# IamJerryXu/Multimodal-Diagnosis-HAM-Spine

Hardware: AMD Instinct MI355X
Metric: training images/sec, ResNet50+BERT-base 224px bs32 (higher is better)
Workload: dtype bf16; 1 GPU; C2: ResNet50 + BERT-base(L=128) + cross-attention FusionModule + MLP head, 224x224, batch 32 per GPU, CE(label_smoothing=0.02), fused AdamW, train-mode BatchNorm and dropout; per_gpu_batch=32, global_batch=32, seq_len=128, params=134897991, parallelism=dp1

## Files before the change

### multimodal-diagnosis-ham-spine_amd/hamspine/csrc/blocks.hip

```cpp
#include <algorithm>
#include <mutex>
#include <unordered_map>
#include <vector>
#include <stdlib.h>
#include "hs_common.h"
#include "pw_stream.h"

namespace hs {

__global__ __launch_bounds__(256) void gather3_kernel(const float* __restrict__ a, const float* __restrict__ b,
                                                      const float* __restrict__ c, float* __restrict__ dst, int n) {
    const int i = blockIdx.x * 256 + threadIdx.x;
    if (i >= 3 * n) return;
    const int w = i / n, k = i - w * n;
    dst[i] = w == 0 ? a[k] : (w == 1 ? b[k] : c[k]);
}

int gemm_impl(const hs_gemm_params* p, hipStream_t stream);
int gemm_stat_rows(const hs_gemm_params* p);
int gemm_bn_finish_rows(const hs_gemm_params* p);
int gemm_tile_rows(const hs_gemm_params* p);
int gemm_bnb_finish_rows(const hs_gemm_params* p);
void gemm_group_set_immediate_hook(int (*fn)(void*), void* ctx);
struct GemmGroup;
GemmGroup* gemm_group_open(hipStream_t s, long long slot);
int gemm_group_add(GemmGroup* g, const hs_gemm_params* p, hipStream_t s, const int* k_cols = nullptr);
bool gemm_group_takes_k_cols();
int gemm_group_flush(GemmGroup* g, hipStream_t s);
bool fused_attention_enabled();
int attention_bwd_fused(const hs_attn_desc& d, const void* q, const void* k, const void* v, const void* dO, void* dq, void* dk,
                        void* dv, const void* P, int ldP, void* scratch, long long scratch_bytes, const void* O, hipStream_t s,
                        const int* cu);
int attention_fwd_fused(const hs_attn_desc& d, const void* q, const void* k, const void* v, void* o, void* P, void* Pd, int ldP,
                        hipStream_t s, const int* cu);
int ln_fwd(int dtype, const void* x, const float* gamma, const float* beta, void* y, float* mean, float* rstd, long long M, int H,
           float eps, hipStream_t s, const int* nrows);
int ln_bwd(int dtype, const void* dy, const void* x, const float* gamma, const float* mean, const float* rstd, void* dx, float* dgamma,
           float* dbeta, float* ws, long long ws_bytes, long long M, int H, hipStream_t s, const int* inv);
int ln_bwd_pre(int dtype, const void* dy, const void* x, const float* gamma, const float* mean, const float* rstd, void* dx,
               float* dgamma, float* dbeta, void* dx_dropped, float* dbias, float p, unsigned long long seed, float* ws,
               long long ws_bytes, long long M, int H, hipStream_t s, const int* inv);
// ... 167 lines not shown
        } else {
            ++m;
        }
    }
    return HS_OK;
}
static int milestones_flush(Run& r) {
    if (r.plan) return HS_OK;
    for (int m = 0; m < g_ms.n; ++m) HS_CHECK_HIP(hipEventRecord(g_ms.ev[m], r.s));
    g_ms.n = 0;
    return HS_OK;
}

static hs_gemm_params gemm_defaults(int dt) {
    hs_gemm_params p;
    memset(&p, 0, sizeof(p));
    p.dtype = dt;
    p.out_dtype = dt;
    p.alpha = 1.f;
    p.batch = 1;
    p.batch_inner = 1;
    return p;
}
static int gemm_splitk(Run& r, hs_gemm_params& p, bool may_defer = false) {
    const int split = hs_gemm_suggest_split(p.M, p.N, p.K, p.dtype);
    const long long mk = r.ws.mark();
    p.split_k = split;
    if (split > 1) p.splitk_ws = (float*)r.ws.alloc(hs_gemm_splitk_ws_bytes(&p));
    const bool defer = may_defer && r.defer_wgrad && p.dtype == HS_BF16;
    if (!r.plan) {
        if (r.ws.overflow) {
            set_error("gemm_splitk: workspace too small");
            return HS_ERR_ARG;
        }
        if (may_defer && (knock() & 1)) {
        } else if (defer) HS_PROPAGATE(gemm_group_add(p.b_kind == HS_B_CONV ? r.grp_conv : r.grp_pw, &p, r.s));
        else HS_PROPAGATE(gemm_impl(&p, r.s));
    }
    if (defer) return HS_OK;
    if (r.plan ? !overlap_enabled() : !r.side) r.ws.release(mk);
    return HS_OK;
}

struct AttnLayout {
    int ldP;
    void *P, *Pd;
    float* S;
    void* dS;
};
static AttnLayout attn_layout(const hs_attn_desc& d, Run& r, bool backward) {
    AttnLayout l;
    const long long BH = (long long)d.B * d.H;
    l.ldP = (int)align_up(d.Lk, 8);
    l.P = r.saved.alloc(BH * d.Lq * l.ldP * esize(d.dtype));
    l.Pd = d.dropout_p > 0.f ? r.saved.alloc(BH * d.Lq * l.ldP * esize(d.dtype)) : l.P;
    l.S = (float*)r.ws.alloc(BH * d.Lq * d.Lk * 4);
    l.dS = backward ? r.ws.alloc(BH * d.Lq * l.ldP * esize(d.dtype)) : nullptr;
    return l;
}
static int attn_check(const hs_attn_desc& d) {
// ... 366 lines not shown
}

struct ConvShape {
    int N, H, W, Cin, Cout, R, stride, pad, P, Q;
};
static ConvShape conv_shape(int N, int H, int W, const hs_conv_bn& c) {
    ConvShape s;
    s.N = N; s.H = H; s.W = W; s.Cin = c.Cin; s.Cout = c.Cout; s.R = c.R; s.stride = c.stride; s.pad = c.pad;
    s.P = (H + 2 * c.pad - c.R) / c.stride + 1;
    s.Q = (W + 2 * c.pad - c.R) / c.stride + 1;
    return s;
}
static hs_conv_geom geom_of(const ConvShape& s) {
    hs_conv_geom g;
    memset(&g, 0, sizeof(g));
    g.N = s.N; g.H = s.H; g.W = s.W; g.C = s.Cin; g.P = s.P; g.Q = s.Q; g.K = s.Cout; g.R = s.R; g.S = s.R;
    g.stride = s.stride; g.pad = s.pad;
    g.row_pitch = s.W * s.Cin;
    g.img_pitch = s.H * g.row_pitch;
    g.qstep = s.stride * s.Cin;
    return g;
}
static bool is_pointwise(const ConvShape& s) { return s.R == 1 && s.stride == 1 && s.pad == 0; }
static bool fused_ln_bwd_enabled() {
    static int v = -1;
    if (v < 0) {
        const char* e = getenv("HAMSPINE_FUSED_LN_BWD");
        v = (e && e[0] == '0') ? 0 : 1;
    }
    return v == 1;
}
static bool grouped_wgrad_enabled() {
    static int v = -1;
    if (v < 0) {
        const char* e = getenv("HAMSPINE_GROUPED_WGRAD");
        v = (e && e[0] == '0') ? 0 : 1;
    }
    return v == 1;
}
static bool bn_mask_from_x_enabled() {
    static int v = -1;
    if (v < 0) {
        const char* e = getenv("HAMSPINE_BN_MASK_FROM_X");
        v = (e && e[0] == '1') ? 1 : 0;
    }
    return v == 1;
// ... 87 lines not shown
struct BnSums {
    const void* c;
    const float *scale, *shift, *mean, *invstd;
    float* partials;
    long long partials_cap;
    int* rows;
    const void* y = nullptr;
    const hs_bn_bwd_params* finish = nullptr;
    int* done = nullptr;
};
static bool bnb_finish_enabled() {
    static const bool on = [] { const char* e = getenv("HAMSPINE_BNB_FINISH"); return e && e[0] == '1'; }();
    return on;
}
static bool fused_bn_bwd_enabled() {
    static int v = -1;
    if (v < 0) {
        const char* e = getenv("HAMSPINE_FUSED_BN_BWD");
        v = (e && e[0] == '0') ? 0 : 1;
    }
    return v == 1;
}
static int conv_dgrad_run(Run& r, const ConvShape& s, const void* dy, const void* w_c, void* dx, const void* residual,
                          const BnSums* bnb = nullptr) {
    hs_gemm_params p = gemm_defaults(r.dt);
    p.M = (int)((long long)s.N * s.H * s.W); p.N = s.Cin; p.K = s.R * s.R * s.Cout;
    p.A = dy; p.B = w_c;
    p.a_elems = (long long)s.N * s.P * s.Q * s.Cout;
    p.b_elems = (long long)s.Cout * s.R * s.R * s.Cin;
    p.D = dx; p.ldd = s.Cin;
    p.residual = residual; p.ldr = s.Cin;
    if (is_pointwise(s)) {
        p.a_kind = HS_A_KC; p.lda = s.Cout;
        p.b_kind = HS_B_RC; p.ldb = s.Cin;
    } else {
        p.a_kind = HS_A_DGRAD; p.b_kind = HS_B_WDGRAD; p.g = geom_of(s);
    }
    if (bnb && bnb->rows) *bnb->rows = 0;
    if (!r.plan && (knock() & 512)) return HS_OK;
    if (bnb && (!residual || bnb->y) && r.dt == HS_BF16 && s.stride == 1 && s.Cin % 8 == 0 && fused_bn_bwd_enabled() && !(knock() & 16)) {
        p.split_k = hs_gemm_suggest_split(p.M, p.N, p.K, p.dtype);
        hs_gemm_params probe = p;
        probe.bnb_x = bnb->c; probe.bnb_scale = bnb->scale; probe.bnb_shift = bnb->shift; probe.bnb_mean = bnb->mean;
        probe.bnb_invstd = bnb->invstd; probe.bnb_partials = bnb->partials; probe.bnb_y = bnb->y;
        const int rows = r.plan ? 0 : gemm_tile_rows(&probe);
        if (bnb->done) *bnb->done = 0;
        if (rows > 0 && ((long long)rows * s.Cin * 2 + 4ll * s.Cin) * 4 <= bnb->partials_cap) {
            p = probe;
            *bnb->rows = rows;
            const int frows = (bnb->finish && bnb->done && bnb_finish_enabled()) ? gemm_bnb_finish_rows(&probe) : 0;
            if (frows > 0 && ((long long)frows * s.Cin * 2 + 4ll * s.Cin) * 4 <= bnb->partials_cap) {
                p.bnb_finish = bnb->finish;
                *bnb->rows = frows;
                *bnb->done = 1;
            }
        }
    }
    if (r.dt == HS_BF16 && s.stride == 1) return gemm_splitk(r, p);
    CALL(r, gemm_impl(&p, r.s));
    return HS_OK;
}
static int conv_wgrad_run(Run& r, const ConvShape& s, const void* dy, const void* x, float* dw) {
    hs_gemm_params p = gemm_defaults(r.dt);
    p.M = s.Cout; p.N = s.R * s.R * s.Cin; p.K = (int)((long long)s.N * s.P * s.Q);
    p.A = dy; p.B = x;
    p.a_elems = (long long)s.N * s.P * s.Q * s.Cout;
    p.b_elems = (long long)s.N * s.H * s.W * s.Cin;
    p.a_kind = HS_A_RC; p.lda = s.Cout;
    p.D = dw; p.ldd = p.N; p.out_dtype = HS_F32;
    if (is_pointwise(s)) {
        p.b_kind = HS_B_RC; p.ldb = s.Cin;
    } else {
        p.b_kind = HS_B_CONV; p.g = geom_of(s);
    }
    return gemm_splitk(r, p, true);
}

struct CastList {
    const float* src[HS_CAST_MAX];
    void* dst[HS_CAST_MAX];
    int64_t n[HS_CAST_MAX];
    int count = 0;
// ... 152 lines not shown
    ResLayout L;
    HS_PROPAGATE(res_layout(r, d, L));
    const int last = d.n_main - 1;
    const int es = esize(r.dt);
    const long long Mout = (long long)d.N * L.main[last].s.P * L.main[last].s.Q;
    const int Cout = d.main[last].Cout;
    void* dres = r.ws.alloc(Mout * Cout * es);
    float* scratch_pg = (float*)r.ws.alloc(2 * 4096 * 4);
    long long max_act = 0;
    for (int i = 0; i < d.n_main; ++i) {
        const StageBuf& b = L.main[i];
        max_act = std::max<long long>(max_act, (long long)d.N * b.s.P * b.s.Q * b.s.Cout);
        max_act = std::max<long long>(max_act, (long long)d.N * b.s.H * b.s.W * b.s.Cin);
    }
    if (d.has_ds) max_act = std::max<long long>(max_act, Mout * Cout);
    void* g_conv[3] = {nullptr, nullptr, nullptr};
    void* g_in[3] = {nullptr, nullptr, nullptr};
    for (int i = 0; i < d.n_main; ++i) {
        const StageBuf& b = L.main[i];
        g_conv[i] = r.ws.alloc((long long)d.N * b.s.P * b.s.Q * b.s.Cout * es);
        if (i > 0) g_in[i] = r.ws.alloc((long long)d.N * b.s.H * b.s.W * b.s.Cin * es);
    }
    void* g_ds = d.has_ds ? r.ws.alloc(Mout * Cout * es) : nullptr;
    void* dx_ds = (d.has_ds && dx) ? r.ws.alloc((long long)d.N * d.H * d.W * d.main[0].Cin * es) : nullptr;
    (void)max_act;
    for (int i = 0; i < d.n_main; ++i) HS_REQUIRE(d.main[i].Cout <= 4096, "resblock: Cout > 4096");
    HS_PROPAGATE(side_setup(r));

    auto bn_backward = [&](const hs_conv_bn& cb, const StageBuf& b, long long M, const void* g_out, const void* y_out,
                           int relu, void* g_in_, void* g_res, int partial_rows = 0, const OwnSums* pre = nullptr,
                           int sums_done = 0) -> int {
        hs_bn_bwd_params q;
        memset(&q, 0, sizeof(q));
        q.partial_rows = partial_rows;
        q.sums_done = partial_rows > 0 ? sums_done : 0;
        q.dtype = r.dt; q.C = cb.Cout; q.M = M;
        q.training = d.training; q.relu = relu;
        q.dy = g_out; q.y = y_out; q.x = b.c;
        q.gamma = cb.gamma; q.save_mean = b.mean; q.save_invstd = b.invstd;
        q.dx = g_in_; q.dres = g_res;
        if (relu && !g_res && bn_mask_from_x_enabled()) {
            q.y = nullptr;
            q.scale = b.scale;
            q.shift = b.shift;
        }
        q.dgamma = cb.dgamma ? cb.dgamma : scratch_pg;
        q.dbeta = cb.dbeta ? cb.dbeta : (scratch_pg ? scratch_pg + 4096 : nullptr);
        q.ws = L.bn_ws; q.ws_bytes = L.bn_ws_bytes;
        if (pre && pre->rows > 0) {
            q.partial_rows = pre->rows;
            q.sums_done = pre->done;
            q.ws = pre->partials; q.ws_bytes = pre->bytes;
        }
        CALLK(r, 16, hs_batchnorm_bwd(&q, r.s));
        return HS_OK;
    };

    HS_PROPAGATE(bn_backward(d.main[last], L.main[last], Mout, dy, y, 1, g_conv[last], dres, 0, own));
    const void* dres_for_x = dres;
    if (d.has_ds) {
        HS_PROPAGATE(bn_backward(d.ds, L.ds, Mout, dres, nullptr, 0, g_ds, nullptr));
        if (d.ds.dw) HS_PROPAGATE(on_side(r, [&]() { return conv_wgrad_run(r, L.ds.s, g_ds, x, d.ds.dw); }));
        if (dx) HS_PROPAGATE(conv_dgrad_run(r, L.ds.s, g_ds, L.ds.w_c, dx_ds, nullptr));
        dres_for_x = dx_ds;
    }
    for (int i = last; i >= 0; --i) {
        const StageBuf& b = L.main[i];
        const void* in = i == 0 ? x : L.main[i - 1].a;
        if (d.main[i].dw) HS_PROPAGATE(on_side(r, [&]() { return conv_wgrad_run(r, b.s, g_conv[i], in, d.main[i].dw); }));
        if (i == 0) {
            if (dx) HS_PROPAGATE(conv_dgrad_run(r, b.s, g_conv[i], b.w_c, dx, dres_for_x, next_bn));
        } else {
            const StageBuf& pb = L.main[i - 1];
            int sum_rows = 0, sum_done = 0;
            const long long Mp = (long long)d.N * pb.s.P * pb.s.Q;
            const hs_conv_bn& pcb = d.main[i - 1];
            hs_bn_bwd_params fin;
            memset(&fin, 0, sizeof(fin));
            fin.dtype = r.dt; fin.C = pcb.Cout; fin.M = Mp; fin.training = d.training;
            fin.gamma = pcb.gamma;
            fin.dgamma = pcb.dgamma ? pcb.dgamma : scratch_pg;
            fin.dbeta = pcb.dbeta ? pcb.dbeta : (scratch_pg ? scratch_pg + 4096 : nullptr);
            BnSums bs = {pb.c, pb.scale, pb.shift, pb.mean, pb.invstd, (float*)L.bn_ws, L.bn_ws_bytes, &sum_rows};
            if (fin.dgamma && fin.dbeta) {
                bs.finish = &fin;
                bs.done = &sum_done;
            }
            HS_PROPAGATE(conv_dgrad_run(r, b.s, g_conv[i], b.w_c, g_in[i], nullptr, &bs));
            HS_PROPAGATE(bn_backward(d.main[i - 1], pb, Mp, g_in[i], pb.a, 1, g_conv[i - 1], nullptr, sum_rows, nullptr, sum_done));
        }
    }
    HS_PROPAGATE(side_join(r));
    RUN_CHECK_ARENAS(r, "resblock_bwd");
    return HS_OK;
// ... 1205 lines not shown
```

### multimodal-diagnosis-ham-spine_amd/hamspine/csrc/gemm.hip

```cpp
#include <atomic>
#include <mutex>
#include <unordered_set>
#include <vector>
#include <stdarg.h>
#include <math.h>
#include <map>
#include <tuple>
#include "gemm_launch.h"
#include "gemm_p8.h"

namespace hs {

static thread_local char g_err[512] = "";
void set_error(const char* fmt, ...) {
    va_list ap;
    va_start(ap, fmt);
    vsnprintf(g_err, sizeof(g_err), fmt, ap);
    va_end(ap);
}
const char* last_error() { return g_err; }

bool lds_attr_needed(const void* fn) {
    static std::mutex mu;
    static std::unordered_set<const void*> seen;
// ... 118 lines not shown
    if (!p || p->dtype != HS_BF16 || p->split_k > 1 || p->batch > 1) return 0;
    {
        int r, t, fm;
        if (conv3_plan(p, &r, &t, &fm)) return p->g.N * t;
    }
    int cfg = (p->a_kind == HS_A_CONV && p->b_kind == HS_B_KC && p->g.C % 64 != 0) ? CFG_STEM : auto_cfg(p, true);
    if (g_dbg_cfg >= 0 && g_dbg_cfg <= CFG_64x64 && cfg != CFG_STEM) cfg = g_dbg_cfg;
    if (g_dbg_cfg >= CFG_256x128 && g_dbg_cfg <= CFG_256x128x32 && !(p->a_kind == HS_A_CONV || p->a_kind == HS_A_DGRAD || p->b_kind == HS_B_CONV)) cfg = g_dbg_cfg;
    return ceil_div(p->M, cfg == CFG_64x64 ? 64 : (cfg == CFG_256x128 || cfg == CFG_256x128x32) ? 256 : 128);
}

static bool bn_finish_variant(int cfg, int combo) {
    return (combo == 0 && (cfg == CFG_64x64 || cfg == CFG_128x64)) || (combo == 3 && (cfg == CFG_64x64 || cfg == CFG_128x64 || cfg == CFG_STEM || cfg == CFG_C3));
}

static int g_pack_spread = -1;
struct Prepared {
    GemmArgs a;
    int cfg, combo, split, batch;
    bool bf16, conv, vec;
    dim3 grid;
    double flops;
};
static int gemm_prepare(const hs_gemm_params* p, hipStream_t stream, Prepared& q, int force_cfg = -1) {
    HS_REQUIRE(p != nullptr, "hs_gemm: null params");
    HS_REQUIRE(p->dtype == HS_F32 || p->dtype == HS_BF16, "hs_gemm: bad dtype %d", p->dtype);
    HS_REQUIRE(p->M > 0 && p->N > 0 && p->K >= 0, "hs_gemm: bad dims %d %d %d", p->M, p->N, p->K);
    HS_REQUIRE(p->A && p->B && p->D, "hs_gemm: null operand");
    const int combo = combo_of(p->a_kind, p->b_kind);
    HS_REQUIRE(combo >= 0, "hs_gemm: unsupported operand kinds (%d,%d)", p->a_kind, p->b_kind);
    const bool bf16 = p->dtype == HS_BF16;
    const int esz = bf16 ? 2 : 4, epc = bf16 ? 8 : 4;
    const int batch = p->batch > 0 ? p->batch : 1;
    const int split = p->split_k > 1 ? p->split_k : 1;
    HS_REQUIRE(!(batch > 1 && split > 1), "hs_gemm: batch and split_k are exclusive");
    HS_REQUIRE((long long)p->a_elems * esz < 0x7fffff00ll && (long long)p->b_elems * esz < 0x7fffff00ll,
               "hs_gemm: operand larger than 2 GiB");
    HS_REQUIRE(p->out_dtype == HS_F32 || p->out_dtype == p->dtype, "hs_gemm: out_dtype must be f32 or the operand type");
    HS_REQUIRE(!p->accumulate || p->out_dtype == HS_F32, "hs_gemm: accumulate needs an f32 output");

    GemmArgs a;
    memset(&a, 0, sizeof(a));
    a.A = (const char*)p->A;
    a.B = (const char*)p->B;
    a.a_bytes = (unsigned long long)p->a_elems * esz;
    a.b_bytes = (unsigned long long)p->b_elems * esz;
    a.lda = p->lda;
// ... 96 lines not shown
            static int parity_on = -1;
            if (parity_on < 0) {
                const char* e = getenv("HAMSPINE_PARITY_DGRAD");
                parity_on = (e && e[0] == '0') ? 0 : 1;
            }
            if (parity_on && bf16 && g.stride == 2 && g.H % 2 == 0 && g.W % 2 == 0 && g.R * g.S <= 15 && split == 1 && batch == 1 &&
                !p->seg_rows && !p->colstats && !p->bnb_partials) {
                a.parity = 1;
                a.quarter = g.N * (g.H / 2) * (g.W / 2);
                a.div_qhw = make_fastdiv((g.H / 2) * (g.W / 2));
                a.div_qw = make_fastdiv(g.W / 2);
            }
        } else {
            HS_REQUIRE(p->K == g.N * g.P * g.Q, "conv wgrad: K != N*P*Q");
            HS_REQUIRE(p->N == g.R * g.S * g.C, "conv wgrad: N != R*S*C");
            HS_REQUIRE(p->M == g.K, "conv wgrad: M != Kout");
            HS_REQUIRE(g.C % epc == 0, "conv wgrad: C %% %d != 0", epc);
            a.div_mhw = make_fastdiv(g.P * g.Q);
            a.div_mw = make_fastdiv(g.Q);
            a.div_sc = make_fastdiv(g.S * g.C);
            a.div_c = make_fastdiv(g.C);
        }
    }

    bool vec = aligned16(p->A) && aligned16(p->B);
    if (p->a_kind == HS_A_KC || p->a_kind == HS_A_RC) vec = vec && (p->lda % epc == 0);
    if (p->b_kind == HS_B_KC || p->b_kind == HS_B_RC) vec = vec && (p->ldb % epc == 0);
    if (batch > 1) vec = vec && (p->a_bs0 % epc == 0) && (p->a_bs1 % epc == 0) && (p->b_bs0 % epc == 0) && (p->b_bs1 % epc == 0);
    if (conv) HS_REQUIRE(vec, "hs_gemm: conv operands must be 16-byte aligned");
    if (bf16) {
        HS_REQUIRE(vec, "hs_gemm(bf16): lda/ldb/batch strides must be multiples of 8 and bases 16-byte aligned");
        const int k8 = (p->K + 7) / 8 * 8;
        if (p->a_kind == HS_A_KC) HS_REQUIRE(p->K % 8 == 0 || p->lda >= k8, "hs_gemm(bf16): A rows need K%%8==0 or zero padding to %d", k8);
        if (p->b_kind == HS_B_KC) HS_REQUIRE(p->K % 8 == 0 || p->ldb >= k8, "hs_gemm(bf16): B rows need K%%8==0 or zero padding to %d", k8);
    }
    {
        const int oesz = a.out_f32 ? 4 : esz;
        bool vs = (p->N % 4 == 0) && (p->ldd % 4 == 0) && ((((uintptr_t)p->D) % (4 * oesz)) == 0);
        if (batch > 1) vs = vs && (p->d_bs0 % 4 == 0) && (p->d_bs1 % 4 == 0);
        if (p->D_preact) vs = vs && ((((uintptr_t)p->D_preact) % (4 * oesz)) == 0);
        if (p->residual) vs = vs && (p->ldr % 4 == 0) && ((((uintptr_t)p->residual) % (4 * oesz)) == 0);
        if (p->mul_src) vs = vs && (p->ldm % 4 == 0) && ((((uintptr_t)p->mul_src) % (4 * esz)) == 0);
        a.vec_store = vs;
        bool v16 = bf16 && !a.out_f32 && (p->N % 8 == 0) && (p->ldd % 8 == 0) && ((((uintptr_t)p->D) & 15) == 0);
        if (batch > 1) v16 = v16 && (p->d_bs0 % 8 == 0) && (p->d_bs1 % 8 == 0);
        if (p->D_preact) v16 = v16 && ((((uintptr_t)p->D_preact) & 15) == 0);
// ... 174 lines not shown
    if (!p || !p->colstats) return 0;
    hs_gemm_params c = *p;
    c.bn_finish = nullptr;
    Prepared q;
    if (gemm_prepare(&c, nullptr, q) != HS_OK) return 0;
    if (!q.bf16 || q.split != 1 || q.batch != 1 || q.a.persist > 0 || !bn_finish_variant(q.cfg, q.combo)) return 0;
    if ((long long)q.a.tiles_n * (1 + stat_groups(q.a.tiles_m)) > kTicketPool) return 0;
    return q.a.tiles_m + stat_groups(q.a.tiles_m);
}

int gemm_bnb_finish_rows(const hs_gemm_params* p) {
    if (!p || !p->bnb_partials) return 0;
    hs_gemm_params c = *p;
    c.bnb_finish = nullptr;
    unsigned char dummy[16];
    if (c.split_k > 1 && !c.splitk_ws) c.splitk_ws = (float*)dummy;
    Prepared q;
    if (gemm_prepare(&c, nullptr, q) != HS_OK) return 0;
    if (!q.bf16 || q.split != 1 || q.batch != 1 || q.a.persist > 0 || !(q.cfg == CFG_64x64 || q.cfg == CFG_128x64)) return 0;
    if ((long long)q.a.tiles_n * (1 + stat_groups(q.a.tiles_m)) > kTicketPool) return 0;
    return q.a.tiles_m + stat_groups(q.a.tiles_m);
}

int gemm_impl(const hs_gemm_params* p, hipStream_t stream) {
    Prepared q;
    HS_PROPAGATE(gemm_prepare(p, stream, q));
    const GemmArgs& a = q.a;
    const int cfg = q.cfg, combo = q.combo, split = q.split, batch = q.batch;
    const bool bf16 = q.bf16, conv = q.conv, vec = q.vec;
    const dim3 grid = q.grid;
    int st;
    ProfRec rec;
    const bool timed = prof_begin(stream, q.flops, (bf16 ? 0 : 2) + (conv ? 1 : 0), rec);
    if (bf16 && cfg == CFG_C3) st = launch_bf16_conv3(a, a.c3_fm, grid, stream);
    else if (bf16 && cfg >= CFG_P8_256 && cfg <= CFG_P8_128) st = launch_bf16_p8(cfg, a, grid, stream);
    else if (bf16) st = conv ? launch_bf16_conv(cfg, combo, a, grid, stream) : launch_bf16_plain(cfg, combo, a, grid, stream);
    else st = conv ? launch_f32_conv(cfg, combo, a, grid, stream) : launch_f32_plain(cfg, combo, vec, a, grid, stream);
    if (timed) {
        rec.M = p->M; rec.N = p->N; rec.K = p->K; rec.combo = combo; rec.cfg = cfg; rec.split = split; rec.batch = batch;
        rec.conv_r = conv ? p->g.R : 0; rec.conv_stride = conv ? p->g.stride : 0;
        prof_end(stream, rec);
    }
    HS_PROPAGATE(st);
    if (split > 1 && !a.tickets) {
        const long long work = (long long)p->M * ((p->N + 3) / 4);
        const int blocks = (int)std::min<long long>((work + 255) / 256, 2048);
        if (bf16) hipLaunchKernelGGL(splitk_reduce_kernel<bf16_t>, dim3(blocks), dim3(256), 0, stream, a);
        else hipLaunchKernelGGL(splitk_reduce_kernel<float>, dim3(blocks), dim3(256), 0, stream, a);
        HS_LAUNCH_CHECK();
// ... 277 lines not shown
```

### multimodal-diagnosis-ham-spine_amd/hamspine/csrc/gemm_core.h

```cpp
#pragma once
#include <type_traits>
#include "hs_common.h"

namespace hs {

struct GemmArgs {
    const char* A;
    const char* B;
    unsigned long long a_bytes, b_bytes;
    int lda, ldb;
    int M, N, K;
    hs_conv_geom g;
    FastDiv div_mhw, div_mw;
    FastDiv div_sc, div_c;
    int batch_inner;
    long long a_bs0, a_bs1, b_bs0, b_bs1, d_bs0, d_bs1;
    int tiles_m, tiles_n;
    int group_m;
    int parity;
    int quarter;
    FastDiv div_qhw, div_qw;
    const float* colscale;
    int res_pre_act;
    float* colstats;
// ... 25 lines not shown
    const char* bnb_x;
    const float *bnb_scale, *bnb_shift, *bnb_mean, *bnb_invstd;
    float* bnb_partials;
    const char* bnb_y;
    const float* bnb_gamma;
    float *bnb_dgamma, *bnb_dbeta;
    float bnb_invm;
    int bnb_train;
    unsigned* bnb_tickets;
    const float *bnf_gamma, *bnf_beta;
    float *bnf_rmean, *bnf_rvar, *bnf_mean, *bnf_invstd, *bnf_scale, *bnf_shift;
    float bnf_eps, bnf_momentum;
    unsigned* bnf_tickets;
    float* rowsum[3];
    int c3_rows, c3_tpi, c3_fm;
    int vec16;
    int epi_generic;
    int dbg;
    unsigned long long* stamps;
    const int* m_rows;
    const int* drop_rows;
    int pack_spread;
    const int* k_cols;
};

#define HS_STAMP(k)                                                                                              \
    do {                                                                                                         \
        if (a.stamps && threadIdx.x == 0)                                                                        \
            a.stamps[((long long)blockIdx.z * gridDim.x + blockIdx.x) * 6 + (k)] = __builtin_readcyclecounter(); \
    } while (0)

__device__ __forceinline__ int parity_class(const GemmArgs& a, int m) {
    return (m >= a.quarter) + (m >= 2 * a.quarter) + (m >= 3 * a.quarter);
}
__device__ __forceinline__ void parity_pixel(const GemmArgs& a, int m, unsigned& n, unsigned& h, unsigned& w) {
    const int cls = parity_class(a, m);
    const unsigned idx = m - cls * a.quarter;
    n = fdiv(idx, a.div_qhw);
    const unsigned ij = idx - n * a.div_qhw.d;
    const unsigned i = fdiv(ij, a.div_qw);
    h = 2 * i + (cls >> 1);
    w = 2 * (ij - i * a.div_qw.d) + (cls & 1);
}
__device__ __forceinline__ long long parity_row(const GemmArgs& a, int m) {
    unsigned n, h, w;
    parity_pixel(a, m, n, h, w);
    return ((long long)n * a.g.H + h) * a.g.W + w;
}


#define HS_GLOBAL __attribute__((address_space(1)))
template <typename T>
__device__ __forceinline__ void load4(const char* base, long long idx, bool vec, int nvalid, float* f) {
    const HS_GLOBAL T* p = (const HS_GLOBAL T*)((const T*)base + idx);
    if (vec) {
        if constexpr (sizeof(T) == 4) {
            f32x4 v = *(const HS_GLOBAL f32x4*)p;
            f[0] = v[0]; f[1] = v[1]; f[2] = v[2]; f[3] = v[3];
        } else {
            u32x2 v = *(const HS_GLOBAL u32x2*)p;
            f[0] = __uint_as_float(v[0] << 16);
            f[1] = __uint_as_float(v[0] & 0xffff0000u);
            f[2] = __uint_as_float(v[1] << 16);
            f[3] = __uint_as_float(v[1] & 0xffff0000u);
        }
    } else {
#pragma unroll
        for (int j = 0; j < 4; ++j) f[j] = j < nvalid ? to_f32(p[j]) : 0.f;
    }
}
template <typename T>
__device__ __forceinline__ void store4(char* base, long long idx, bool vec, int nvalid, const float* f) {
    HS_GLOBAL T* p = (HS_GLOBAL T*)((T*)base + idx);
    if (vec) {
        if constexpr (sizeof(T) == 4) {
            f32x4 v = {f[0], f[1], f[2], f[3]};
            *(HS_GLOBAL f32x4*)p = v;
        } else {
            bf16x4 v = {(bf16_t)f[0], (bf16_t)f[1], (bf16_t)f[2], (bf16_t)f[3]};
            *(HS_GLOBAL bf16x4*)p = v;
        }
    } else {
#pragma unroll
        for (int j = 0; j < 4; ++j)
            if (j < nvalid) p[j] = from_f32<T>(f[j]);
    }
}

enum {
    EPI_BIAS = 1, EPI_COLSCALE = 2, EPI_MUL_GELU = 4, EPI_MUL_RELU = 8, EPI_SEG = 16, EPI_PREACT = 32, EPI_RES_PRE = 64,
    EPI_RES_POST = 128, EPI_RELU = 256, EPI_GELU = 512, EPI_DROP = 1024, EPI_OUT_F32 = 2048, EPI_ACCUM = 4096, EPI_VEC = 8192,
    EPI_PARITY = 16384, EPI_VEC16 = 32768
};
__device__ __forceinline__ unsigned epi_flags(const GemmArgs& a) {
    unsigned f = 0;
    if (a.bias) f |= EPI_BIAS;
    if (a.colscale) f |= EPI_COLSCALE;
    if (a.mul_mode == HS_MUL_GELU_GRAD) f |= EPI_MUL_GELU;
    else if (a.mul_mode != HS_MUL_NONE) f |= EPI_MUL_RELU;
    if (a.seg_rows > 0) f |= EPI_SEG;
    if (a.D_preact) f |= EPI_PREACT;
    if (a.residual) f |= a.res_pre_act ? EPI_RES_PRE : EPI_RES_POST;
    if (a.act == HS_ACT_RELU) f |= EPI_RELU;
    else if (a.act == HS_ACT_GELU) f |= EPI_GELU;
    if (a.drop_thresh) f |= EPI_DROP;
    if (a.out_f32) f |= EPI_OUT_F32;
    if (a.accumulate) f |= EPI_ACCUM;
    if (a.vec_store) f |= EPI_VEC;
    if (a.parity) f |= EPI_PARITY;
    if (a.vec16) f |= EPI_VEC16;
    return f;
}

template <typename T, int CF = -1, bool FULL = false, bool DEFER = false>
__device__ __forceinline__ void epilogue4(const GemmArgs& a, unsigned rt_flags, long long dbase, int z, int m, int n,
                                          float* v, float* pv = nullptr, int md_in = -1) {
    if constexpr (!FULL) {
        if (m >= a.M || n >= a.N) return;
    }
    const unsigned fl = CF >= 0 ? (unsigned)CF : rt_flags;
    const long long mr = (fl & EPI_PARITY) ? parity_row(a, m) : (long long)m;
    const int nvalid = FULL ? 4 : min(4, a.N - n);
    const bool vec = FULL ? true : ((fl & EPI_VEC) && nvalid == 4);
    const bool out_f32 = fl & EPI_OUT_F32;
#pragma unroll
// ... 46 lines not shown
    if (fl & EPI_RELU) {
#pragma unroll
        for (int j = 0; j < 4; ++j) v[j] = fmaxf(v[j], 0.f);
    } else if (fl & EPI_GELU) {
#pragma unroll
        for (int j = 0; j < 4; ++j) v[j] = gelu_fwd_t<T>(v[j]);
    }
    if (fl & EPI_DROP) {
        const unsigned long long md = md_in >= 0 ? (unsigned long long)md_in
                                      : a.drop_rows ? (unsigned long long)((const HS_GLOBAL int*)a.drop_rows)[m] : (unsigned long long)m;
        const unsigned long long q = ((unsigned long long)z * a.M + md) * (unsigned long long)a.N + n;
        if ((q & 3) == 0) {
            float sc[4];
            dropout_scale4(a.drop_seed, q, a.drop_thresh, a.drop_inv_keep, sc);
#pragma unroll
            for (int j = 0; j < 4; ++j) v[j] *= sc[j];
        } else {
#pragma unroll
            for (int j = 0; j < 4; ++j) v[j] *= dropout_scale(a.drop_seed, q + j, a.drop_thresh, a.drop_inv_keep);
        }
    }
    if (fl & EPI_RES_POST) {
        float r[4];
        const long long ridx = dbase + mr * a.ldr + n;
        if (out_f32) load4<float>(a.residual, ridx, vec, nvalid, r);
        else load4<T>(a.residual, ridx, vec, nvalid, r);
#pragma unroll
        for (int j = 0; j < 4; ++j) v[j] += r[j];
    }
    if constexpr (DEFER) return;
    if (out_f32) {
        if (fl & EPI_ACCUM) {
            float o[4];
            load4<float>(Dp, didx, vec, nvalid, o);
#pragma unroll
            for (int j = 0; j < 4; ++j) v[j] += o[j];
        }
        store4<float>(Dp, didx, vec, nvalid, v);
    } else {
        store4<T>(Dp, didx, vec, nvalid, v);
    }
}

template <int CPR>
__device__ __forceinline__ int kc_swz(int r) {
    constexpr int RPB = 16 / CPR;
    const int j = (r / RPB) % CPR;
    return CPR == 4 ? ((CPR - j) & (CPR - 1)) : j;
}
// ... 696 lines not shown
            stage_dma(0, k_of(0));
#pragma unroll
            for (int q = 1; q < NS; ++q)
                if (q < ntiles) stage_dma(q, k_of(q));
        }
    };
    constexpr int PFM = BNS ? FM : 1, PFN = BNS ? FN : 1;
    u32x2 pf_c[PFM][PFN], pf_y[PFM][PFN], pf_r[PFM][PFN];
    bool pf = false;
    if constexpr (BNS) {
        if (a.bnb_partials && a.split_k == 1) {
            pf = true;
            const bool wy = a.bnb_y != nullptr, wr = wy && a.residual != nullptr;
#pragma unroll
            for (int i = 0; i < FM; ++i)
#pragma unroll
                for (int j = 0; j < FN; ++j) {
                    const int m = m0 + wm * WM + i * 16 + l15, n = n0 + wn * WN + j * 16 + 4 * g;
                    const bool live = m < a.M && n < a.N;
                    pf_c[i][j] = pf_y[i][j] = pf_r[i][j] = u32x2{0u, 0u};
                    if (live) {
                        pf_c[i][j] = *(const HS_GLOBAL u32x2*)((const HS_GLOBAL T*)a.bnb_x + (long long)m * a.ldd + n);
                        if (wy) pf_y[i][j] = *(const HS_GLOBAL u32x2*)((const HS_GLOBAL T*)a.bnb_y + (long long)m * a.ldd + n);
                        if (wr) pf_r[i][j] = *(const HS_GLOBAL u32x2*)((const HS_GLOBAL T*)a.residual + (long long)m * a.ldr + n);
                    }
                }
        }
    }
    constexpr int NDR = (WM + 63) / 64;
    int drow_v[NDR];
#pragma unroll
    for (int j = 0; j < NDR; ++j) drow_v[j] = 0;
    const bool have_drow = a.drop_rows != nullptr && a.drop_thresh != 0;
    if (have_drow) {
#pragma unroll
        for (int j = 0; j < NDR; ++j) drow_v[j] = ((const HS_GLOBAL int*)a.drop_rows)[min(m0 + wm * WM + j * 64 + lane, a.M - 1)];
    }
    issue_prologue();
    HS_STAMP(1);
    if (a.stamps && threadIdx.x == 0) a.stamps[((long long)blockIdx.z * gridDim.x + blockIdx.x) * 6] = t_entry;
    const int pstride = PS ? a.persist : 0;
    int vb = bx;
    bool first_tile = true;
    for (;;) {
#pragma unroll
    for (int i = 0; i < FM; ++i)
#pragma unroll
// ... 286 lines not shown
                    const bool live = nok && m < argM;
                    auto unpack = [](const u32x2 v, float* f) {
                        f[0] = __uint_as_float(v[0] << 16);
                        f[1] = __uint_as_float(v[0] & 0xffff0000u);
                        f[2] = __uint_as_float(v[1] << 16);
                        f[3] = __uint_as_float(v[1] & 0xffff0000u);
                    };
                    if (pf) {
                        unpack(pf_c[i][j], cv);
                        if (from_y) {
                            unpack(pf_y[i][j], yv);
                            if (res_consumed) {
                                float rv[4];
                                unpack(pf_r[i][j], rv);
#pragma unroll
                                for (int e = 0; e < 4; ++e) acc[i][j][e] += rv[e];
                            }
                        }
                    } else {
                    if (live) load4<T>(a.bnb_x, (long long)m * a.ldd + n, true, 4, cv);
                    if (from_y && live) {
                        load4<T>(a.bnb_y, (long long)m * a.ldd + n, true, 4, yv);
                        if (res_consumed) {
                            float rv[4];
                            load4<T>(a.residual, (long long)m * a.ldr + n, true, 4, rv);
#pragma unroll
                            for (int e = 0; e < 4; ++e) acc[i][j][e] += rv[e];
                        }
                    }
                    }
#pragma unroll
                    for (int e = 0; e < 4; ++e) {
                        const float gq = (float)(bf16_t)acc[i][j][e];
                        const bool on = from_y ? yv[e] > 0.f : fmaf(cv[e], sc[e], sh[e]) > 0.f;
                        const float dz = (live && on) ? gq : 0.f;
                        u[e] += dz;
                        w[e] = fmaf(dz, (cv[e] - mu[e]) * is[e], w[e]);
                    }
                }
#pragma unroll
                for (int e = 0; e < 4; ++e) {
#pragma unroll
                    for (int o = 1; o < 16; o <<= 1) {
                        u[e] += __shfl_xor(u[e], o, 64);
                        w[e] += __shfl_xor(w[e], o, 64);
                    }
                    s1[j][e] = u[e];
                    s2[j][e] = w[e];
// ... 27 lines not shown
                    o[0] = t1;
                    o[1] = t2;
                }
            }
            __syncthreads();
            if (a.bnb_tickets) {
                const int ng = stat_groups(a.tiles_m);
                unsigned* ticket = ng ? a.bnb_tickets + a.tiles_n + tn * ng + tm / kStatGroup : a.bnb_tickets + tn;
                asm volatile("s_waitcnt vmcnt(0)" ::: "memory");
                __syncthreads();
                if (tid == 0) bnb_drawn = (int)__hip_atomic_fetch_add(ticket, 1u, __ATOMIC_RELAXED, __HIP_MEMORY_SCOPE_AGENT);
            }
        }
    }
    const int em0 = m0, en0 = n0;
    const int nvb = vb + pstride;
    const bool more = PS && pstride > 0 && nvb < a.tiles_m * a.tiles_n;
    if (more) {
        asm volatile("s_waitcnt lgkmcnt(0)" ::: "memory");
        __builtin_amdgcn_s_barrier();
        setup_tile(nvb);
        issue_prologue();
    }
    const unsigned epi_e = res_consumed ? (epi & ~(unsigned)EPI_RES_POST) : epi;
    int mdrop[FM];
#pragma unroll
    for (int i = 0; i < FM; ++i) mdrop[i] = have_drow ? __shfl(drow_v[(i * 16) / 64], (i * 16 + l15) & 63, 64) : -1;
    const bool full = !a.epi_generic && (epi & EPI_VEC) && em0 + BM <= argM && en0 + BN <= argN;
    bool done = false;
    const int ze = split_k > 1 ? 0 : z;
    if (full) {
        done = true;
#define HS_EPI_CASE(F) case (F): run_epilogue<T, (F), true, FM, FN, WM, WN>(a, epi_e, acc, em0, en0, wm, wn, l15, g, d_boff, ze, mdrop); break
        const bool v16 = epi_e & EPI_VEC16;
        const unsigned key = epi_e & ~EPI_VEC16;
        if (!v16 && !(key & EPI_OUT_F32)) done = false;
        else switch (key) {
            HS_EPI_CASE(EPI_VEC);
            HS_EPI_CASE(EPI_VEC | EPI_BIAS);
            HS_EPI_CASE(EPI_VEC | EPI_BIAS | EPI_GELU | EPI_PREACT);
            HS_EPI_CASE(EPI_VEC | EPI_BIAS | EPI_RES_POST);
            HS_EPI_CASE(EPI_VEC | EPI_BIAS | EPI_DROP | EPI_RES_POST);
            HS_EPI_CASE(EPI_VEC | EPI_MUL_GELU);
            HS_EPI_CASE(EPI_VEC | EPI_RES_POST);
            HS_EPI_CASE(EPI_VEC | EPI_OUT_F32);
            HS_EPI_CASE(EPI_VEC | EPI_OUT_F32 | EPI_SEG);
            HS_EPI_CASE(EPI_VEC | EPI_PARITY);
            HS_EPI_CASE(EPI_VEC | EPI_BIAS | EPI_COLSCALE | EPI_RELU);
            HS_EPI_CASE(EPI_VEC | EPI_BIAS | EPI_COLSCALE);
            HS_EPI_CASE(EPI_VEC | EPI_BIAS | EPI_COLSCALE | EPI_RELU | EPI_RES_PRE);
            default: done = false;
        }
#undef HS_EPI_CASE
    }
    if (!done) run_epilogue<T, -1, false, FM, FN, WM, WN>(a, epi_e, acc, em0, en0, wm, wn, l15, g, d_boff, ze, mdrop);
    HS_STAMP(4);
    if constexpr (BNF && !PS) {
        if (a.bnf_tickets) bnf_handoff<WGM * 128, BN>(a, smem, tid, tm, tn, en0, bnf_drawn);
    }
    if constexpr (BNS && !PS) {
        if (a.bnb_partials && a.bnb_tickets) bnb_handoff<WGM * 128, BN>(a, smem, tid, tm, tn, en0, bnb_drawn);
    }
    if (!more) break;
    vb = nvb;
    first_tile = false;
    }
}
// ... 261 lines not shown
```

### multimodal-diagnosis-ham-spine_amd/hamspine/csrc/gemm_p8.h

```cpp
#pragma once
#include "gemm_core.h"

namespace hs {

template <int N>
__device__ __forceinline__ void wait_vmcnt() {
    asm volatile("s_waitcnt vmcnt(%0)" ::"n"(N) : "memory");
}

template <int BM, int BN, int WGM, int WGN, bool RS, bool STAG, bool DIAG = false, int TAG = 0>
__device__ __forceinline__ void gemm_bf16_p8_body(const GemmArgs& a, const int bx) {
    typedef bf16_t T;
    constexpr int BK = 64, NW = WGM * WGN;
    constexpr int WM = BM / WGM, WN = BN / WGN;
    constexpr int QM = WM / 2, QN = WN / 2;
    constexpr int FMQ = QM / 16, FNQ = QN / 16;
    constexpr int FM = 2 * FMQ, FN = 2 * FNQ;
    constexpr int A_SLOT = (BM / 2) * BK * 2, B_SLOT = (BN / 2) * BK * 2;
    constexpr int BUF = 2 * A_SLOT + 2 * B_SLOT;
    constexpr int NA = A_SLOT / 1024 / NW, NB = B_SLOT / 1024 / NW;
    static_assert(QM % 16 == 0 && QN % 16 == 0 && NA >= 1 && NB >= 1 && A_SLOT % (1024 * NW) == 0 && B_SLOT % (1024 * NW) == 0, "tile / wave shape");
    static_assert(3 * NA + 3 * NB <= 63, "vmcnt field");
    extern __shared__ __attribute__((aligned(16))) char smem[];
    typedef __attribute__((address_space(3))) char lds_char;
// ... 242 lines not shown
        HS_EPI_CASE(EPI_VEC | EPI_OUT_F32);
        HS_EPI_CASE(EPI_VEC | EPI_OUT_F32 | EPI_SEG);
        default: break;
    }
#undef HS_EPI_CASE
}

inline bool p8_epilogue_supported(const GemmArgs& a) {
    unsigned f = 0;
    if (a.bias) f |= EPI_BIAS;
    if (a.colscale) f |= EPI_COLSCALE;
    if (a.mul_mode == HS_MUL_GELU_GRAD) f |= EPI_MUL_GELU;
    else if (a.mul_mode != HS_MUL_NONE) f |= EPI_MUL_RELU;
    if (a.seg_rows > 0) f |= EPI_SEG;
    if (a.D_preact) f |= EPI_PREACT;
    if (a.residual) f |= a.res_pre_act ? EPI_RES_PRE : EPI_RES_POST;
    if (a.act == HS_ACT_RELU) f |= EPI_RELU;
    else if (a.act == HS_ACT_GELU) f |= EPI_GELU;
    if (a.drop_thresh) f |= EPI_DROP;
    if (a.out_f32) f |= EPI_OUT_F32;
    if (a.accumulate) f |= EPI_ACCUM;
    if (a.vec_store) f |= EPI_VEC;
    if (a.parity) f |= EPI_PARITY;
    if (a.epi_generic || a.alpha != 1.f) return false;
    if (!(f & EPI_OUT_F32) && !a.vec16) return false;
    switch (f) {
        case EPI_VEC: case EPI_VEC | EPI_BIAS: case EPI_VEC | EPI_BIAS | EPI_GELU | EPI_PREACT: case EPI_VEC | EPI_BIAS | EPI_RES_POST:
        case EPI_VEC | EPI_BIAS | EPI_DROP | EPI_RES_POST: case EPI_VEC | EPI_MUL_GELU: case EPI_VEC | EPI_RES_POST:
        case EPI_VEC | EPI_OUT_F32: case EPI_VEC | EPI_OUT_F32 | EPI_SEG:
            return true;
    }
    return false;
}

template <bool RS>
__global__ __launch_bounds__(512) void gemm_bf16_p8_256_kernel(const GemmArgs a) {
    gemm_bf16_p8_body<256, 256, 2, 4, RS, true>(a, blockIdx.x);
}
__global__ __launch_bounds__(512) void gemm_bf16_p8_256_diag_kernel(const GemmArgs a);
template <bool RS>
__global__ __launch_bounds__(512) void gemm_bf16_p8_grouped_kernel(const GemmArgs* __restrict__ list, const int* __restrict__ first_wg, int n) {
    const int bid = blockIdx.x, lane = threadIdx.x & 63;
    const int lo = lane < n ? first_wg[lane] : 0x7fffffff;
    const int p = __builtin_amdgcn_readfirstlane(__popcll(__ballot(lo <= bid)) - 1);
    const int local = bid - __builtin_amdgcn_readfirstlane(first_wg[p]);
    gemm_bf16_p8_body<256, 256, 2, 4, RS, true, false, 1>(list[p], local);
}
// ... 11 lines not shown
```

### multimodal-diagnosis-ham-spine_amd/hamspine/csrc/hs_common.h

```cpp
#pragma once
#include <hip/hip_runtime.h>
#include <stdint.h>
#include <stdio.h>
#include <string.h>
#include "../../../include/hamspine.h"

namespace hs {

void set_error(const char* fmt, ...);

#define HS_CHECK_HIP(expr)                                                                   \
    do {                                                                                     \
        hipError_t _e = (expr);                                                              \
        if (_e != hipSuccess) {                                                              \
            hs::set_error("%s:%d: %s -> %s", __FILE__, __LINE__, #expr, hipGetErrorString(_e)); \
            return HS_ERR_HIP;                                                               \
        }                                                                                    \
    } while (0)

#define HS_REQUIRE(cond, ...)                                                                \
    do {                                                                                     \
        if (!(cond)) {                                                                       \
            hs::set_error(__VA_ARGS__);                                                      \
            return HS_ERR_ARG;                                                               \
// ... 94 lines not shown
struct FastDiv {
    unsigned d, mul, shr;
};
inline FastDiv make_fastdiv(unsigned d) {
    FastDiv f;
    f.d = d;
    if (d <= 1) {
        f.mul = 0;
        f.shr = 0;
        return f;
    }
    unsigned lg = 0;
    while ((1u << lg) < d) ++lg;
    unsigned p = 31 + lg;
    unsigned long long m = ((1ull << p) + d - 1) / d;
    f.mul = (unsigned)m;
    f.shr = p - 32;
    return f;
}
__device__ __forceinline__ unsigned fdiv(unsigned n, const FastDiv& f) {
    return f.d <= 1 ? n : (__umulhi(n, f.mul) >> f.shr);
}

__device__ __forceinline__ unsigned hash_u32(unsigned long long seed, unsigned long long idx) {
    unsigned long long z = seed + idx * 0x9E3779B97F4A7C15ull;
    z = (z ^ (z >> 30)) * 0xBF58476D1CE4E5B9ull;
    z = (z ^ (z >> 27)) * 0x94D049BB133111EBull;
    z = z ^ (z >> 31);
    return (unsigned)(z >> 32);
}
__device__ __forceinline__ unsigned mix32(unsigned x) {
    x ^= x >> 16;
    x *= 0x7feb352du;
    x ^= x >> 15;
    x *= 0x846ca68bu;
    x ^= x >> 16;
    return x;
}
__device__ __forceinline__ u32x2 dropout_bits4(unsigned long long seed, unsigned long long q) {
    const unsigned s0 = (unsigned)seed, s1 = (unsigned)(seed >> 32);
    const unsigned x = (unsigned)q * 0x9E3779B1u + s0 + (unsigned)(q >> 32) * 0x85EBCA77u;
    u32x2 r;
    r[0] = mix32(x ^ s1);
    r[1] = mix32(r[0] + 0x6C8E9CF5u + s1);
    return r;
}
// ... 80 lines not shown
```

Before: 3159 images/s.

## Compute strided 1x1 downsample dgrad compactly and gather it as a residual

In the ResNet bottleneck backward pass, the stride-2 1x1 downsample convolution's data gradient is now computed as a plain GEMM over the P x Q output pixels instead of the full H x W input grid. Three quarters of that grid would be zeros, so this skips that work and the matching writes. The compact result is then added into the first main conv's dgrad epilogue through a new residual-gather path, which maps each output row to its even-pixel source row or zero. In exchange the epilogue gains extra index arithmetic, the fast p8 epilogue is disabled when gather is active, and the compact GEMM bypasses the split-k path.

```diff
diff --git a/multimodal-diagnosis-ham-spine_amd/hamspine/csrc/blocks.hip b/multimodal-diagnosis-ham-spine_amd/hamspine/csrc/blocks.hip
--- a/multimodal-diagnosis-ham-spine_amd/hamspine/csrc/blocks.hip
+++ b/multimodal-diagnosis-ham-spine_amd/hamspine/csrc/blocks.hip
@@ -16,7 +16,7 @@
     dst[i] = w == 0 ? a[k] : (w == 1 ? b[k] : c[k]);
 }
 
-int gemm_impl(const hs_gemm_params* p, hipStream_t stream);
+int gemm_impl(const hs_gemm_params* p, hipStream_t stream, const ResGather* rg = nullptr);
 int gemm_stat_rows(const hs_gemm_params* p);
 int gemm_bn_finish_rows(const hs_gemm_params* p);
 int gemm_tile_rows(const hs_gemm_params* p);
@@ -230,7 +230,7 @@
     p.batch_inner = 1;
     return p;
 }
-static int gemm_splitk(Run& r, hs_gemm_params& p, bool may_defer = false) {
+static int gemm_splitk(Run& r, hs_gemm_params& p, bool may_defer = false, const ResGather* rg = nullptr) {
     const int split = hs_gemm_suggest_split(p.M, p.N, p.K, p.dtype);
     const long long mk = r.ws.mark();
     p.split_k = split;
@@ -243,7 +243,7 @@
         }
         if (may_defer && (knock() & 1)) {
         } else if (defer) HS_PROPAGATE(gemm_group_add(p.b_kind == HS_B_CONV ? r.grp_conv : r.grp_pw, &p, r.s));
-        else HS_PROPAGATE(gemm_impl(&p, r.s));
+        else HS_PROPAGATE(gemm_impl(&p, r.s, rg));
     }
     if (defer) return HS_OK;
     if (r.plan ? !overlap_enabled() : !r.side) r.ws.release(mk);
@@ -656,6 +656,11 @@
     return g;
 }
 static bool is_pointwise(const ConvShape& s) { return s.R == 1 && s.stride == 1 && s.pad == 0; }
+static bool ds_compact(int dt, const ConvShape& s) {
+    if (dt != HS_BF16 || s.R != 1 || s.stride != 2 || s.pad != 0) return false;
+    const char* e = getenv("HAMSPINE_DS_COMPACT");
+    return !(e && e[0] == '0');
+}
 static bool fused_ln_bwd_enabled() {
     static int v = -1;
     if (v < 0) {
@@ -789,8 +794,20 @@
     return v == 1;
 }
 static int conv_dgrad_run(Run& r, const ConvShape& s, const void* dy, const void* w_c, void* dx, const void* residual,
-                          const BnSums* bnb = nullptr) {
+                          const BnSums* bnb = nullptr, const ResGather* rg = nullptr, bool compact = false) {
     hs_gemm_params p = gemm_defaults(r.dt);
+    if (compact) {
+        p.M = (int)((long long)s.N * s.P * s.Q); p.N = s.Cin; p.K = s.Cout;
+        p.A = dy; p.B = w_c;
+        p.a_elems = (long long)p.M * s.Cout;
+        p.b_elems = (long long)s.Cout * s.Cin;
+        p.a_kind = HS_A_KC; p.lda = s.Cout;
+        p.b_kind = HS_B_RC; p.ldb = s.Cin;
+        p.D = dx; p.ldd = s.Cin;
+        if (!r.plan && (knock() & 512)) return HS_OK;
+        CALL(r, gemm_impl(&p, r.s));
+        return HS_OK;
+    }
     p.M = (int)((long long)s.N * s.H * s.W); p.N = s.Cin; p.K = s.R * s.R * s.Cout;
     p.A = dy; p.B = w_c;
     p.a_elems = (long long)s.N * s.P * s.Q * s.Cout;
@@ -823,8 +840,8 @@
             }
         }
     }
-    if (r.dt == HS_BF16 && s.stride == 1) return gemm_splitk(r, p);
-    CALL(r, gemm_impl(&p, r.s));
+    if (r.dt == HS_BF16 && s.stride == 1) return gemm_splitk(r, p, false, rg);
+    CALL(r, gemm_impl(&p, r.s, rg));
     return HS_OK;
 }
 static int conv_wgrad_run(Run& r, const ConvShape& s, const void* dy, const void* x, float* dw) {
@@ -1023,7 +1040,10 @@
         if (i > 0) g_in[i] = r.ws.alloc((long long)d.N * b.s.H * b.s.W * b.s.Cin * es);
     }
     void* g_ds = d.has_ds ? r.ws.alloc(Mout * Cout * es) : nullptr;
-    void* dx_ds = (d.has_ds && dx) ? r.ws.alloc((long long)d.N * d.H * d.W * d.main[0].Cin * es) : nullptr;
+    const bool ds_cmp = d.has_ds && dx && ds_compact(r.dt, L.ds.s);
+    const long long ds_rows = (ds_cmp && !r.plan) ? (long long)d.N * L.ds.s.P * L.ds.s.Q : (long long)d.N * d.H * d.W;
+    void* dx_ds = (d.has_ds && dx) ? r.ws.alloc(ds_rows * d.main[0].Cin * es) : nullptr;
+    const ResGather ds_rg = {d.H, d.W};
     (void)max_act;
     for (int i = 0; i < d.n_main; ++i) HS_REQUIRE(d.main[i].Cout <= 4096, "resblock: Cout > 4096");
     HS_PROPAGATE(side_setup(r));
@@ -1062,7 +1082,7 @@
     if (d.has_ds) {
         HS_PROPAGATE(bn_backward(d.ds, L.ds, Mout, dres, nullptr, 0, g_ds, nullptr));
         if (d.ds.dw) HS_PROPAGATE(on_side(r, [&]() { return conv_wgrad_run(r, L.ds.s, g_ds, x, d.ds.dw); }));
-        if (dx) HS_PROPAGATE(conv_dgrad_run(r, L.ds.s, g_ds, L.ds.w_c, dx_ds, nullptr));
+        if (dx) HS_PROPAGATE(conv_dgrad_run(r, L.ds.s, g_ds, L.ds.w_c, dx_ds, nullptr, nullptr, nullptr, ds_cmp));
         dres_for_x = dx_ds;
     }
     for (int i = last; i >= 0; --i) {
@@ -1070,7 +1090,7 @@
         const void* in = i == 0 ? x : L.main[i - 1].a;
         if (d.main[i].dw) HS_PROPAGATE(on_side(r, [&]() { return conv_wgrad_run(r, b.s, g_conv[i], in, d.main[i].dw); }));
         if (i == 0) {
-            if (dx) HS_PROPAGATE(conv_dgrad_run(r, b.s, g_conv[i], b.w_c, dx, dres_for_x, next_bn));
+            if (dx) HS_PROPAGATE(conv_dgrad_run(r, b.s, g_conv[i], b.w_c, dx, dres_for_x, next_bn, ds_cmp ? &ds_rg : nullptr));
         } else {
             const StageBuf& pb = L.main[i - 1];
             int sum_rows = 0, sum_done = 0;
diff --git a/multimodal-diagnosis-ham-spine_amd/hamspine/csrc/gemm.hip b/multimodal-diagnosis-ham-spine_amd/hamspine/csrc/gemm.hip
--- a/multimodal-diagnosis-ham-spine_amd/hamspine/csrc/gemm.hip
+++ b/multimodal-diagnosis-ham-spine_amd/hamspine/csrc/gemm.hip
@@ -164,7 +164,7 @@
     dim3 grid;
     double flops;
 };
-static int gemm_prepare(const hs_gemm_params* p, hipStream_t stream, Prepared& q, int force_cfg = -1) {
+static int gemm_prepare(const hs_gemm_params* p, hipStream_t stream, Prepared& q, int force_cfg = -1, const ResGather* rg = nullptr) {
     HS_REQUIRE(p != nullptr, "hs_gemm: null params");
     HS_REQUIRE(p->dtype == HS_F32 || p->dtype == HS_BF16, "hs_gemm: bad dtype %d", p->dtype);
     HS_REQUIRE(p->M > 0 && p->N > 0 && p->K >= 0, "hs_gemm: bad dims %d %d %d", p->M, p->N, p->K);
@@ -307,6 +307,19 @@
             a.div_c = make_fastdiv(g.C);
         }
     }
+    if (rg) {
+        HS_REQUIRE(bf16 && p->out_dtype == HS_BF16 && p->residual && !p->residual_before_act && batch == 1 && p->seg_rows <= 0 &&
+                       (combo <= 2 || combo == 4) && rg->H > 0 && rg->W > 0 && p->M % (rg->H * rg->W) == 0,
+                   "hs_gemm: a compact residual needs a bf16 GEMM or data-gradient convolution over whole H x W images, added after the activation");
+        if (conv) HS_REQUIRE(p->g.H == rg->H && p->g.W == rg->W, "hs_gemm: compact residual: grid mismatch");
+        else {
+            a.div_mhw = make_fastdiv(rg->H * rg->W);
+            a.div_mw = make_fastdiv(rg->W);
+        }
+        a.res_gather = 1;
+        a.res_p = (rg->H + 1) / 2;
+        a.res_q = (rg->W + 1) / 2;
+    }
 
     bool vec = aligned16(p->A) && aligned16(p->B);
     if (p->a_kind == HS_A_KC || p->a_kind == HS_A_RC) vec = vec && (p->lda % epc == 0);
@@ -527,9 +540,9 @@
     return q.a.tiles_m + stat_groups(q.a.tiles_m);
 }
 
-int gemm_impl(const hs_gemm_params* p, hipStream_t stream) {
+int gemm_impl(const hs_gemm_params* p, hipStream_t stream, const ResGather* rg = nullptr) {
     Prepared q;
-    HS_PROPAGATE(gemm_prepare(p, stream, q));
+    HS_PROPAGATE(gemm_prepare(p, stream, q, -1, rg));
     const GemmArgs& a = q.a;
     const int cfg = q.cfg, combo = q.combo, split = q.split, batch = q.batch;
     const bool bf16 = q.bf16, conv = q.conv, vec = q.vec;
diff --git a/multimodal-diagnosis-ham-spine_amd/hamspine/csrc/gemm_core.h b/multimodal-diagnosis-ham-spine_amd/hamspine/csrc/gemm_core.h
--- a/multimodal-diagnosis-ham-spine_amd/hamspine/csrc/gemm_core.h
+++ b/multimodal-diagnosis-ham-spine_amd/hamspine/csrc/gemm_core.h
@@ -71,6 +71,8 @@
     const int* drop_rows;
     int pack_spread;
     const int* k_cols;
+    int res_gather;
+    int res_p, res_q;
 };
 
 #define HS_STAMP(k)                                                                                              \
@@ -95,6 +97,15 @@
     unsigned n, h, w;
     parity_pixel(a, m, n, h, w);
     return ((long long)n * a.g.H + h) * a.g.W + w;
+}
+__device__ __forceinline__ long long res_gather_row(const GemmArgs& a, int m, bool parity) {
+    if (parity) return m < a.quarter ? (long long)m : -1ll;
+    const unsigned n = fdiv(m, a.div_mhw);
+    const unsigned hw = m - n * a.div_mhw.d;
+    const unsigned h = fdiv(hw, a.div_mw);
+    const unsigned w = hw - h * a.div_mw.d;
+    if ((h | w) & 1) return -1ll;
+    return ((long long)n * a.res_p + (h >> 1)) * a.res_q + (w >> 1);
 }
 
 
@@ -139,7 +150,8 @@
 enum {
     EPI_BIAS = 1, EPI_COLSCALE = 2, EPI_MUL_GELU = 4, EPI_MUL_RELU = 8, EPI_SEG = 16, EPI_PREACT = 32, EPI_RES_PRE = 64,
     EPI_RES_POST = 128, EPI_RELU = 256, EPI_GELU = 512, EPI_DROP = 1024, EPI_OUT_F32 = 2048, EPI_ACCUM = 4096, EPI_VEC = 8192,
-    EPI_PARITY = 16384, EPI_VEC16 = 32768
+    EPI_PARITY = 16384, EPI_VEC16 = 32768,
+    EPI_RES_GATHER = 65536
 };
 __device__ __forceinline__ unsigned epi_flags(const GemmArgs& a) {
     unsigned f = 0;
@@ -150,6 +162,7 @@
     if (a.seg_rows > 0) f |= EPI_SEG;
     if (a.D_preact) f |= EPI_PREACT;
     if (a.residual) f |= a.res_pre_act ? EPI_RES_PRE : EPI_RES_POST;
+    if (a.residual && a.res_gather) f |= EPI_RES_GATHER;
     if (a.act == HS_ACT_RELU) f |= EPI_RELU;
     else if (a.act == HS_ACT_GELU) f |= EPI_GELU;
     if (a.drop_thresh) f |= EPI_DROP;
@@ -242,9 +255,16 @@
     }
     if (fl & EPI_RES_POST) {
         float r[4];
-        const long long ridx = dbase + mr * a.ldr + n;
-        if (out_f32) load4<float>(a.residual, ridx, vec, nvalid, r);
-        else load4<T>(a.residual, ridx, vec, nvalid, r);
+        if (fl & EPI_RES_GATHER) {
+            const long long rr = res_gather_row(a, m, fl & EPI_PARITY);
+#pragma unroll
+            for (int j = 0; j < 4; ++j) r[j] = 0.f;
+            if (rr >= 0) load4<T>(a.residual, rr * a.ldr + n, vec, nvalid, r);
+        } else {
+            const long long ridx = dbase + mr * a.ldr + n;
+            if (out_f32) load4<float>(a.residual, ridx, vec, nvalid, r);
+            else load4<T>(a.residual, ridx, vec, nvalid, r);
+        }
 #pragma unroll
         for (int j = 0; j < 4; ++j) v[j] += r[j];
     }
@@ -987,7 +1007,10 @@
                     if (live) {
                         pf_c[i][j] = *(const HS_GLOBAL u32x2*)((const HS_GLOBAL T*)a.bnb_x + (long long)m * a.ldd + n);
                         if (wy) pf_y[i][j] = *(const HS_GLOBAL u32x2*)((const HS_GLOBAL T*)a.bnb_y + (long long)m * a.ldd + n);
-                        if (wr) pf_r[i][j] = *(const HS_GLOBAL u32x2*)((const HS_GLOBAL T*)a.residual + (long long)m * a.ldr + n);
+                        if (wr) {
+                            const long long rr = a.res_gather ? res_gather_row(a, m, false) : (long long)m;
+                            if (rr >= 0) pf_r[i][j] = *(const HS_GLOBAL u32x2*)((const HS_GLOBAL T*)a.residual + rr * a.ldr + n);
+                        }
                     }
                 }
         }
@@ -1320,8 +1343,9 @@
                     if (from_y && live) {
                         load4<T>(a.bnb_y, (long long)m * a.ldd + n, true, 4, yv);
                         if (res_consumed) {
-                            float rv[4];
-                            load4<T>(a.residual, (long long)m * a.ldr + n, true, 4, rv);
+                            float rv[4] = {0.f, 0.f, 0.f, 0.f};
+                            const long long rr = a.res_gather ? res_gather_row(a, m, false) : (long long)m;
+                            if (rr >= 0) load4<T>(a.residual, rr * a.ldr + n, true, 4, rv);
 #pragma unroll
                             for (int e = 0; e < 4; ++e) acc[i][j][e] += rv[e];
                         }
@@ -1395,7 +1419,7 @@
         setup_tile(nvb);
         issue_prologue();
     }
-    const unsigned epi_e = res_consumed ? (epi & ~(unsigned)EPI_RES_POST) : epi;
+    const unsigned epi_e = res_consumed ? (epi & ~(unsigned)(EPI_RES_POST | EPI_RES_GATHER)) : epi;
     int mdrop[FM];
 #pragma unroll
     for (int i = 0; i < FM; ++i) mdrop[i] = have_drow ? __shfl(drow_v[(i * 16) / 64], (i * 16 + l15) & 63, 64) : -1;
@@ -1416,6 +1440,7 @@
             HS_EPI_CASE(EPI_VEC | EPI_BIAS | EPI_DROP | EPI_RES_POST);
             HS_EPI_CASE(EPI_VEC | EPI_MUL_GELU);
             HS_EPI_CASE(EPI_VEC | EPI_RES_POST);
+            HS_EPI_CASE(EPI_VEC | EPI_RES_POST | EPI_RES_GATHER);
             HS_EPI_CASE(EPI_VEC | EPI_OUT_F32);
             HS_EPI_CASE(EPI_VEC | EPI_OUT_F32 | EPI_SEG);
             HS_EPI_CASE(EPI_VEC | EPI_PARITY);
diff --git a/multimodal-diagnosis-ham-spine_amd/hamspine/csrc/gemm_p8.h b/multimodal-diagnosis-ham-spine_amd/hamspine/csrc/gemm_p8.h
--- a/multimodal-diagnosis-ham-spine_amd/hamspine/csrc/gemm_p8.h
+++ b/multimodal-diagnosis-ham-spine_amd/hamspine/csrc/gemm_p8.h
@@ -288,7 +288,7 @@
     if (a.accumulate) f |= EPI_ACCUM;
     if (a.vec_store) f |= EPI_VEC;
     if (a.parity) f |= EPI_PARITY;
-    if (a.epi_generic || a.alpha != 1.f) return false;
+    if (a.epi_generic || a.alpha != 1.f || a.res_gather) return false;
     if (!(f & EPI_OUT_F32) && !a.vec16) return false;
     switch (f) {
         case EPI_VEC: case EPI_VEC | EPI_BIAS: case EPI_VEC | EPI_BIAS | EPI_GELU | EPI_PREACT: case EPI_VEC | EPI_BIAS | EPI_RES_POST:
diff --git a/multimodal-diagnosis-ham-spine_amd/hamspine/csrc/hs_common.h b/multimodal-diagnosis-ham-spine_amd/hamspine/csrc/hs_common.h
--- a/multimodal-diagnosis-ham-spine_amd/hamspine/csrc/hs_common.h
+++ b/multimodal-diagnosis-ham-spine_amd/hamspine/csrc/hs_common.h
@@ -140,6 +140,10 @@
     return f.d <= 1 ? n : (__umulhi(n, f.mul) >> f.shr);
 }
 
+struct ResGather {
+    int H, W;
+};
+
 __device__ __forceinline__ unsigned hash_u32(unsigned long long seed, unsigned long long idx) {
     unsigned long long z = seed + idx * 0x9E3779B97F4A7C15ull;
     z = (z ^ (z >> 30)) * 0xBF58476D1CE4E5B9ull;
```

New measurement: 3213 images/s (median of 6 runs). +1.7%, better.
